# MCG-NJU/LinK

Measured on AMD Instinct MI355X. Metric: voxels/s through one LinK (3x7)^3 block, 100k active voxels C=64, higher is better.
Workload: dtype f32

## Files before the change

link_amd/csrc/dense_common.h:

```cpp
#pragma once
#include <limits.h>

#include "elk_common.h"

namespace link {

typedef int v4i_t __attribute__((ext_vector_type(4)));

#define DC_OOB 0xFFFFFFF0u
#ifndef DC_PROF
#define DC_PROF 0
#endif
#define DC_PROF_PTR(p) do { if (!DC_PROF) (p) = nullptr; } while (0)
#define DC_NOW() (DC_PROF == 2 ? __builtin_amdgcn_s_memrealtime() : __builtin_amdgcn_s_memtime())
#ifndef DC_ST_AUX
#define DC_ST_AUX 16
#endif
__device__ __forceinline__ __amdgpu_buffer_rsrc_t dc_rsrc(const void *base, uint32_t bytes) {
  return __builtin_amdgcn_make_buffer_rsrc(const_cast<void *>(base), 0, bytes, 0x00020000);
}
__device__ __forceinline__ void st16(__amdgpu_buffer_rsrc_t r, uint32_t byte_off, float4 v) {
  const v4i_t x = {__builtin_bit_cast(int, v.x), __builtin_bit_cast(int, v.y), __builtin_bit_cast(int, v.z),
                   __builtin_bit_cast(int, v.w)};
  __builtin_amdgcn_raw_buffer_store_b128(x, r, byte_off, 0, DC_ST_AUX);
}
__device__ __forceinline__ void st16i(__amdgpu_buffer_rsrc_t r, uint32_t byte_off, int4 v) {
  const v4i_t x = {v.x, v.y, v.z, v.w};
  __builtin_amdgcn_raw_buffer_store_b128(x, r, byte_off, 0, 0);
}
__device__ __forceinline__ void st4i(__amdgpu_buffer_rsrc_t r, uint32_t byte_off, int v) {
  __builtin_amdgcn_raw_buffer_store_b32(v, r, byte_off, 0, 0);
}
template <bool COH>
__device__ __forceinline__ void st16i_c(__amdgpu_buffer_rsrc_t r, uint32_t byte_off, int4 v) {
  const v4i_t x = {v.x, v.y, v.z, v.w};
  __builtin_amdgcn_raw_buffer_store_b128(x, r, byte_off, 0, COH ? 16 : 0);
}
template <bool COH>
__device__ __forceinline__ void st4i_c(__amdgpu_buffer_rsrc_t r, uint32_t byte_off, int v) {
  __builtin_amdgcn_raw_buffer_store_b32(v, r, byte_off, 0, COH ? 16 : 0);
}
template <bool COH>
__device__ __forceinline__ int4 ld16i_c(__amdgpu_buffer_rsrc_t r, const int4 *base, uint32_t idx) {
  if constexpr (COH) {
    const v4i_t x = __builtin_amdgcn_raw_buffer_load_b128(r, idx * 16u, 0, 16);
    return make_int4(x.x, x.y, x.z, x.w);
  } else {
    return base[idx];
  }
}
template <bool COH>
__device__ __forceinline__ int ld4i_c(__amdgpu_buffer_rsrc_t r, const uint32_t *base, uint32_t idx) {
  if constexpr (COH) return __builtin_amdgcn_raw_buffer_load_b32(r, idx * 4u, 0, 16);
  else return (int)base[idx];
}

#define DC_STATS_SLOTS 16
__device__ __forceinline__ void dc_index_stats_flush(int32_t *stats, int n_in, int n_first, int mx) {
  __shared__ int s_part[16][3];
#pragma unroll
  for (int o = 32; o > 0; o >>= 1) {
    n_in += __shfl_xor(n_in, o, 64);
    n_first += __shfl_xor(n_first, o, 64);
    mx = max(mx, __shfl_xor(mx, o, 64));
  }
  const int lane = (int)(threadIdx.x & 63), wave = (int)(threadIdx.x >> 6);
  if (lane == 0) { s_part[wave][0] = n_in; s_part[wave][1] = n_first; s_part[wave][2] = mx; }
  __syncthreads();
  if (threadIdx.x == 0) {
    int a = 0, f = 0, m = 0;
    for (int w = 0; w < (int)(blockDim.x >> 6); w++) { a += s_part[w][0]; f += s_part[w][1]; m = max(m, s_part[w][2]); }
    int32_t *slot = stats + (blockIdx.x % DC_STATS_SLOTS) * 16;
    if (a) atomicAdd(&slot[0], a);
    if (f) atomicAdd(&slot[1], f);
    if (m) atomicMax(&slot[2], m);
  }
}

#ifndef DC_THETA_BOUND
#define DC_THETA_BOUND 1
#endif
__device__ __forceinline__ void dc_coord_absmax(const link_dc_grid_t &g, float coord_div, float &ax, float &ay, float &az) {
  float a[3];
#pragma unroll
  for (int k = 0; k < 3; k++) {
    const float lo = (float)g.lo[k] * (float)g.s, hi = ((float)g.lo[k] + (float)g.dim[k]) * (float)g.s;
    a[k] = fmaxf(fabsf(lo), fabsf(hi)) / coord_div;
  }
  ax = a[0]; ay = a[1]; az = a[2];
}
__device__ __forceinline__ bool dc_theta_leaves_fast_range(float ax, float ay, float az, float w0, float w1, float w2, float alpha) {
  const float b = (fabsf(w0) * ax + fabsf(w1) * ay + fabsf(w2) * az) * fabsf(alpha) * 1.01f;
  return !(b < 32768.0f);
}

__device__ __forceinline__ int dc_cell(const link_dc_grid_t &g, int ux, int uy, int uz, int ub) {
  return ((ub * g.pdim[0] + ux + 1) * g.pdim[1] + uy + 1) * g.pdim[2] + uz + 1;
}

#define DC_INL 4
__device__ __forceinline__ uint32_t dc_slot(const link_dc_grid_t &g, int pcell, int rank) {
  return rank < DC_INL ? (uint32_t)pcell * DC_INL + (uint32_t)rank
                       : (uint32_t)g.vp * DC_INL + (uint32_t)pcell * (uint32_t)(g.k - DC_INL) + (uint32_t)(rank - DC_INL);
}

template <bool STATS, bool COH = false>
__device__ __forceinline__ void dc_index_body(const int4 *__restrict__ coords, int64_t n, const link_dc_grid_t &g,
                                              uint32_t *__restrict__ cnt, int4 *__restrict__ slots,
                                              int32_t *__restrict__ vcell, int32_t *__restrict__ hdr, int bid, int nblk,
                                              int nthr, int &st_in, int &st_first, int &st_max) {
  const __amdgpu_buffer_rsrc_t r_slots = dc_rsrc(slots, (uint32_t)((int64_t)g.vp * g.k * 16));
  const __amdgpu_buffer_rsrc_t r_cnt = dc_rsrc(cnt, (uint32_t)(g.vp * 4));
  if (bid == 0 && threadIdx.x == 0) hdr[LINK_HDR_NVALID] = (int32_t)n;
  for (int64_t v = (int64_t)bid * nthr + threadIdx.x; v < n; v += (int64_t)nblk * nthr) {
    const int4 rc = coords[v];
    const unsigned ux = (unsigned)(floordiv(rc.x, g.s) - g.lo[0]), uy = (unsigned)(floordiv(rc.y, g.s) - g.lo[1]);
    const unsigned uz = (unsigned)(floordiv(rc.z, g.s) - g.lo[2]), ub = (unsigned)(rc.w - g.lo[3]);
    const bool inside = ux < (unsigned)g.dim[0] && uy < (unsigned)g.dim[1] && uz < (unsigned)g.dim[2] &&
                        ub < (unsigned)g.dim[3];
    if (!inside) atomicOr(&hdr[LINK_HDR_STATUS_ACC], 1);
    const int pcell = inside ? dc_cell(g, (int)ux, (int)uy, (int)uz, (int)ub) : 0;
    const int rank = __builtin_amdgcn_raw_ptr_buffer_atomic_add_i32(1, r_cnt, pcell ? (uint32_t)pcell * 4u : DC_OOB, 0, 0);
    const bool full = pcell != 0 && rank >= g.k;
    if (full) atomicOr(&hdr[LINK_HDR_STATUS_ACC], 2);
    const bool keep = pcell != 0 && !full;
    st16i_c<COH>(r_slots, keep ? dc_slot(g, pcell, rank) * 16u : DC_OOB, make_int4(rc.x, rc.y, rc.z, (int)v));
    vcell[v] = keep ? pcell : 0;
    if (STATS) { st_in += pcell != 0; st_first += (pcell != 0 && rank == 0); st_max = max(st_max, pcell != 0 ? rank + 1 : 0); }
  }
}

#define DC_SID_INL 8
__device__ __forceinline__ uint32_t dc_sid_off(const link_dc_grid_t &g, int pcell, int rank) {
  const int kk = g.k > DC_SID_INL ? g.k - DC_SID_INL : 0;
  return rank < DC_SID_INL ? (uint32_t)pcell * DC_SID_INL + (uint32_t)rank
                           : (uint32_t)g.vp * DC_SID_INL + (uint32_t)pcell * (uint32_t)kk + (uint32_t)(rank - DC_SID_INL);
}

template <int N>
__device__ __forceinline__ void wait_vmcnt() {
  asm volatile("s_waitcnt vmcnt(%0)" ::"n"(N) : "memory");
}

static inline bool dc_width_ok(int c) { return c == 16 || c == 32 || c == 64 || c == 128; }

}
```

link_amd/csrc/dense_fused_impl.h:

```cpp
#pragma once
#include <type_traits>

#include "dense_gather.h"
#include "dense_io.h"

namespace DC_IO_NS {
using namespace link;

#include "dense_k1_impl.h"

template <int C, int OP, int NB, bool PIPE, bool WB = true>
static int launch_k1p(const link_dc_buffers_t *b, const link_dc_grid_t &g, const link_elk_desc_t &d, int64_t n,
                     bool warm, hipStream_t st) {
  using K = dc_k1_cfg<C, OP>;
  const int64_t vi = (int64_t)g.dim[0] * g.dim[1] * g.dim[2] * g.dim[3];
  int64_t waves = (int64_t)(b->tune.k1_wgs > 0 ? b->tune.k1_wgs : 512) * 4;
  int cpw = (int)((vi + waves - 1) / waves);
  if (cpw < 1) cpw = 1;
  const int64_t wgs = (vi + (int64_t)cpw * K::NW - 1) / ((int64_t)cpw * K::NW);
  int k1_pad = b->tune.k1_lds_pad;
  k1_pad = k1_pad < 0 ? 0 : (k1_pad > 16384 ? 16384 : k1_pad);
  const int lds_k1 = K::LDS_BYTES + k1_pad <= 160 * 1024 ? K::LDS_BYTES + k1_pad : K::LDS_BYTES;
  if (lds_k1 > 64 * 1024)
    (void)hipFuncSetAttribute(reinterpret_cast<const void *>(&k_dc_premix_modsum<C, OP, NB, PIPE, WB>),
                              hipFuncAttributeMaxDynamicSharedMemorySize, lds_k1);
  hipLaunchKernelGGL((k_dc_premix_modsum<C, OP, NB, PIPE, WB>), dim3((unsigned)wgs), dim3(64 * K::NW), lds_k1, st, b->feats,
                     reinterpret_cast<int4 *>(b->slots), b->cnt, b->cell_n, b->w_pre, b->pre_ln_w, b->pre_ln_b,
                     b->w_pos, b->alpha, d.cg, d.coord_div, d.eps, n, g, cpw, warm, b->S, b->fin, b->hdr,
                     reinterpret_cast<unsigned long long *>(b->tune.k1_dbg));
  return check_launch("link_dc_premix_modsum");
}

template <int C, int OP, int NB>
static int launch_k1(const link_dc_buffers_t *b, const link_dc_grid_t &g, const link_elk_desc_t &d, int64_t n,
                     bool warm, bool wb, hipStream_t st) {
  if constexpr (C == 64 && NB == 2 && OP != LINK_OP_COSX) {
    if (!wb) return launch_k1p<C, OP, NB, false, false>(b, g, d, n, warm, st);
  }
  return launch_k1p<C, OP, NB, false>(b, g, d, n, warm, st);
}

template <int C, int OP>
static int dispatch_k1_nb(const link_dc_buffers_t *b, const link_dc_grid_t &g, const link_elk_desc_t &d, int64_t n,
                          bool warm, bool wb, hipStream_t st) {
  constexpr int T = C / 16;
  int nb = (d.cg % 16 == 0) ? d.cg / 16 : T;
  if (nb > T) nb = T;
  if (nb == T) return launch_k1<C, OP, T>(b, g, d, n, warm, wb, st);
  if (T >= 2 && nb == T / 2) return launch_k1<C, OP, (T >= 2 ? T / 2 : 1)>(b, g, d, n, warm, wb, st);
  if (T >= 4 && nb == T / 4) return launch_k1<C, OP, (T >= 4 ? T / 4 : 1)>(b, g, d, n, warm, wb, st);
  return launch_k1<C, OP, T>(b, g, d, n, warm, wb, st);
}

template <int C>
static int dispatch_k1_op(const link_dc_buffers_t *b, const link_dc_grid_t &g, const link_elk_desc_t &d, int64_t n,
                          bool warm, bool wb, hipStream_t st) {
  switch (d.op) {
    case LINK_OP_COS: return dispatch_k1_nb<C, LINK_OP_COS>(b, g, d, n, warm, wb, st);
    case LINK_OP_SIN: return dispatch_k1_nb<C, LINK_OP_SIN>(b, g, d, n, warm, wb, st);
    default: return dispatch_k1_nb<C, LINK_OP_COSX>(b, g, d, n, warm, wb, st);
  }
}

#include "dense_fused_mm_impl.h"

template <int LPR, int OP, bool PAIR, bool DIV>
__global__ void __launch_bounds__(256) k_dc_demod(const float *__restrict__ A_, const float *__restrict__ fin,
                                                  const int4 *__restrict__ coords, const int32_t *__restrict__ vcell,
                                                  const float *__restrict__ w_pos, const float *__restrict__ alpha,
                                                  const float *__restrict__ ln_w, const float *__restrict__ ln_b, int c,
                                                  int cg, float coord_div, float eps, int64_t n, int64_t a_rows,
                                                  void *__restrict__ out) {
  constexpr int P = (OP == LINK_OP_COSX) ? 3 : 2;
  constexpr int G = 64 / LPR;
  const int lane = threadIdx.x & 63;
  const int li = lane & (LPR - 1);
  const int ch0 = 4 * li;
  const bool hi = PAIR && (li >= LPR / 2);
  const int ra = P * c * 4;
  const __amdgpu_buffer_rsrc_t r_A = dc_rsrc(A_, (uint32_t)(a_rows * ra));
  const __amdgpu_buffer_rsrc_t r_fin = dc_rsrc(fin, (uint32_t)(n * c * 4));
  const __amdgpu_buffer_rsrc_t r_out = dc_rsrc(out, (uint32_t)(n * c * IO_BYTES));
  float w0[4], w1[4], w2[4], al[4], gw[4], gb[4];
#pragma unroll
  for (int e = 0; e < 4; e++) {
    const int ch = ch0 + e, tc = ch % cg;
    w0[e] = w_pos[3 * tc + 0]; w1[e] = w_pos[3 * tc + 1]; w2[e] = w_pos[3 * tc + 2];
    al[e] = alpha ? alpha[tc] : 1.0f;
    gw[e] = ln_w[ch]; gb[e] = ln_b[ch];
  }
  const float inv_c = 1.0f / (float)c;
  const int64_t npair = (n + 1) >> 1;
  const int64_t ngroups = (int64_t)gridDim.x * 4 * G;
  int64_t p = ((int64_t)blockIdx.x * 4 + (threadIdx.x >> 6)) * G + lane / LPR;
  if (p >= npair) return;
  auto ld_meta = [&](int64_t pp, int4 &ca, int4 &cb, int &va, int &vb) {
    const int64_t q = pp < npair ? pp : npair - 1;
    const int64_t ia = 2 * q, ib = (2 * q + 1 < n) ? 2 * q + 1 : 2 * q;
    ca = coords[ia]; cb = coords[ib];
    va = vcell[ia]; vb = vcell[ib];
  };
  auto ld_rows = [&](int va, int vb, v4i_t (&ra_)[P], v4i_t (&rb_)[P]) {
#pragma unroll
    for (int pp = 0; pp < P; pp++) {
      ra_[pp] = __builtin_amdgcn_raw_buffer_load_b128(r_A, (uint32_t)va * (uint32_t)ra + (uint32_t)((pp * c + ch0) * 4), 0, 0);
      rb_[pp] = __builtin_amdgcn_raw_buffer_load_b128(r_A, (uint32_t)vb * (uint32_t)ra + (uint32_t)((pp * c + ch0) * 4), 0, 0);
    }
  };
  int4 c0a, c0b, c1a, c1b;
  int v0a, v0b, v1a, v1b;
  v4i_t a0[P], b0[P];
  ld_meta(p, c0a, c0b, v0a, v0b);
  ld_rows(v0a, v0b, a0, b0);
  ld_meta(p + ngroups, c1a, c1b, v1a, v1b);
  for (; p < npair; p += ngroups) {
    v4i_t a1[P], b1[P];
    ld_rows(v1a, v1b, a1, b1);
    int4 c2a, c2b;
    int v2a, v2b;
    ld_meta(p + 2 * ngroups, c2a, c2b, v2a, v2b);
    const bool hasB = 2 * p + 1 < n;
    v4i_t fx = {0, 0, 0, 0}, fy = {0, 0, 0, 0};
    if (OP == LINK_OP_COSX) {
      fx = __builtin_amdgcn_raw_buffer_load_b128(r_fin, (uint32_t)(2 * p) * (uint32_t)(c * 4) + (uint32_t)(ch0 * 4), 0, 0);
      fy = __builtin_amdgcn_raw_buffer_load_b128(r_fin, hasB ? (uint32_t)(2 * p + 1) * (uint32_t)(c * 4) + (uint32_t)(ch0 * 4) : DC_OOB, 0, 0);
    }
    float nvA[4], nvB[4], sA = 0.f, sB = 0.f;
    float thA[4], thB[4];
    bool big = false;
    {
      const bool swapped = PAIR && hi && hasB;
      float xa = (float)(swapped ? c0b.x : c0a.x), ya = (float)(swapped ? c0b.y : c0a.y), za = (float)(swapped ? c0b.z : c0a.z);
      float xb = (float)c0b.x, yb = (float)c0b.y, zb = (float)c0b.z;
      if (DIV) { xa = xa / coord_div; ya = ya / coord_div; za = za / coord_div; xb = xb / coord_div; yb = yb / coord_div; zb = zb / coord_div; }
#pragma unroll
      for (int e = 0; e < 4; e++) {
        thA[e] = theta_of(xa, ya, za, w0[e], w1[e], w2[e], al[e]);
        thB[e] = PAIR ? thA[e] : theta_of(xb, yb, zb, w0[e], w1[e], w2[e], al[e]);
        big |= !(fabsf(thA[e]) < 32768.0f) || !(fabsf(thB[e]) < 32768.0f);
      }
    }
    float snA[4], csA[4], snB[4], csB[4];
    if (__builtin_expect(__any(big), 0)) {
#pragma unroll
      for (int e = 0; e < 4; e++) {
        sincos_nocall(thA[e], snA[e], csA[e]);
        if (PAIR) { snB[e] = snA[e]; csB[e] = csA[e]; } else sincos_nocall(thB[e], snB[e], csB[e]);
      }
    } else {
#pragma unroll
      for (int e = 0; e < 4; e++) {
        sincos_small(thA[e], snA[e], csA[e]);
        if (PAIR) { snB[e] = snA[e]; csB[e] = csA[e]; } else sincos_small(thB[e], snB[e], csB[e]);
      }
    }
    if (PAIR) {
      const bool swapped = hi && hasB;
#pragma unroll
      for (int e = 0; e < 4; e++) {
        const float sn = snA[e], cs = csA[e];
        const float so = partner<LPR>(sn), co = partner<LPR>(cs);
        snA[e] = swapped ? so : sn; csA[e] = swapped ? co : cs;
        snB[e] = hi ? sn : so;      csB[e] = hi ? cs : co;
      }
    }
#pragma unroll
    for (int e = 0; e < 4; e++) {
      const float A0 = __int_as_float(a0[0][e]), A1 = __int_as_float(a0[1][e]);
      const float B0 = __int_as_float(b0[0][e]), B1 = __int_as_float(b0[1][e]);
      if (OP == LINK_OP_SIN) {
        nvA[e] = __fsub_rn(__fmul_rn(A0, csA[e]), __fmul_rn(A1, snA[e]));
        nvB[e] = __fsub_rn(__fmul_rn(B0, csB[e]), __fmul_rn(B1, snB[e]));
      } else {
        nvA[e] = __fadd_rn(__fmul_rn(A0, csA[e]), __fmul_rn(A1, snA[e]));
        nvB[e] = __fadd_rn(__fmul_rn(B0, csB[e]), __fmul_rn(B1, snB[e]));
      }
      if (OP == LINK_OP_COSX) {
        nvA[e] = __fadd_rn(nvA[e], __fsub_rn(__int_as_float(a0[P - 1][e]), link_mul_rn(__int_as_float(fx[e]), thA[e])));
        nvB[e] = __fadd_rn(nvB[e], __fsub_rn(__int_as_float(b0[P - 1][e]), link_mul_rn(__int_as_float(fy[e]), thB[e])));
      }
      sA += nvA[e]; sB += nvB[e];
    }
    sA = grp_sum<LPR>(sA);
    sB = grp_sum<LPR>(sB);
    const float meanA = sA * inv_c, meanB = sB * inv_c;
    float qA = 0.f, qB = 0.f;
#pragma unroll
    for (int e = 0; e < 4; e++) {
// ... 780 lines not shown
```

link_amd/csrc/dense_k1_impl.h:

```cpp
#pragma once

#ifndef DC_K1_LCAP
#define DC_K1_LCAP 352
#endif
#ifndef DC_K1_NW
#define DC_K1_NW 4
#endif
#ifndef DC_K1_ABL
#define DC_K1_ABL 0
#endif
#ifndef DC_K1_SPLIT
#define DC_K1_SPLIT 1
#endif
#ifndef DC_K2_ABL
#define DC_K2_ABL 0
#endif
#ifndef DC_K2_SECOND_ROUND
#define DC_K2_SECOND_ROUND 1
#endif
#ifndef DC_K2_PIPE_READS
#define DC_K2_PIPE_READS 0
#endif
#ifndef DC_K1_MFMA32
#define DC_K1_MFMA32 1
#endif
#ifndef DC_K1_SUMB
#define DC_K1_SUMB 8
#endif
#ifndef DC_K1_SWAP_SUMS
#define DC_K1_SWAP_SUMS 1
#endif
#ifndef DC_K1_LATE_PUBLISH
#define DC_K1_LATE_PUBLISH 0
#endif
__device__ __forceinline__ float dc_k1_sum_groups(float v) {
#if DC_K1_SWAP_SUMS
  float a = v, b = v;
  asm volatile("s_nop 1\n\tv_permlane32_swap_b32 %0, %1" : "+v"(a), "+v"(b));
  a += b;
  b = a;
  asm volatile("s_nop 1\n\tv_permlane16_swap_b32 %0, %1" : "+v"(a), "+v"(b));
  return a + b;
#else
  v += __shfl_xor(v, 16, 64);
  v += __shfl_xor(v, 32, 64);
  return v;
#endif
}

template <int C, int OP>
struct dc_k1_cfg {
  static constexpr int T = C / 16;
  static constexpr int P = op_parts<OP>::value;
  static constexpr int LDW = C + 4;
  static constexpr int RB = P * C * 4;
  static constexpr int XROW = RB + 16;
  static constexpr int RGL = P * C / 4;
  static constexpr int RGS = RGL <= 8 ? 8 : (RGL <= 16 ? 16 : (RGL <= 32 ? 32 : 64));
  static constexpr int RG = 64 / RGS;
  static constexpr int LCAP = DC_K1_LCAP;
  static constexpr int LDH = 2 * C + 8;
  static constexpr int WIMG_BYTES = DC_K1_SPLIT ? C * LDH * 2 : C * LDW * 4;
  static constexpr int W_BYTES = WIMG_BYTES + (2 * C + 4 * C) * 4;
  static constexpr int LIST_OFF = 0;
  static constexpr int SCELL_OFF = LCAP * 16;
  static constexpr int X_OFF = SCELL_OFF + LCAP * 4;
  static constexpr int WAVE_BYTES = X_OFF + 16 * XROW;
  static constexpr int NW = DC_K1_NW;
  static constexpr int LDS_BYTES = W_BYTES + NW * WAVE_BYTES;
};


#ifndef DC_K1_WAVES
#define DC_K1_WAVES 2
#endif
__device__ __forceinline__ int dc_k1_cell_of(const link_dc_grid_t &g, int chunk, int nrem, int lane) {
  const int q = chunk + (lane < nrem ? lane : 0);
  const int Dx = g.dim[0], Dy = g.dim[1], Dz = g.dim[2];
  const int z = q % Dz;
  int t = q / Dz;
  const int y = t % Dy;
  t /= Dy;
  return dc_cell(g, t % Dx, y, z, t / Dx);
}

template <bool COH = false>
__device__ __forceinline__ void dc_k1_prefetch(int &pc_f, int &nv_f, int4 &rf0, int4 &rf1, int4 &rf2, int4 &rf3,
                                               const link_dc_grid_t &g, const int4 *__restrict__ slots,
                                               const uint32_t *__restrict__ csrc, int c_begin, int c_end, int lane) {
  pc_f = 0; nv_f = 0;
  rf0 = make_int4(0, 0, 0, 0); rf1 = rf0; rf2 = rf0; rf3 = rf0;
  if (c_begin < c_end) {
    pc_f = dc_k1_cell_of(g, c_begin, (c_end - c_begin < 64) ? c_end - c_begin : 64, lane);
    const __amdgpu_buffer_rsrc_t r_slots = dc_rsrc(slots, (uint32_t)((int64_t)g.vp * g.k * 16));
    const __amdgpu_buffer_rsrc_t r_c = dc_rsrc(csrc, (uint32_t)(g.vp * 4));
    rf0 = ld16i_c<COH>(r_slots, slots, (uint32_t)pc_f * DC_INL + 0); rf1 = ld16i_c<COH>(r_slots, slots, (uint32_t)pc_f * DC_INL + 1);
    rf2 = ld16i_c<COH>(r_slots, slots, (uint32_t)pc_f * DC_INL + 2); rf3 = ld16i_c<COH>(r_slots, slots, (uint32_t)pc_f * DC_INL + 3);
    nv_f = ld4i_c<COH>(r_c, csrc, (uint32_t)pc_f);
  }
}

template <int C, int OP>
__device__ __forceinline__ void dc_k1_stage(char *smem_raw, const float *__restrict__ w_pre, const float *__restrict__ ln_w,
                                            const float *__restrict__ ln_b, const float *__restrict__ w_pos,
                                            const float *__restrict__ alpha, int cg, float coord_div, const link_dc_grid_t &g,
                                            int tid, bool &w_big, bool &th_big) {
  using K = dc_k1_cfg<C, OP>;
  constexpr int LDW = K::LDW;
  float *w_lds = reinterpret_cast<float *>(smem_raw);
  float *ln_lds = reinterpret_cast<float *>(smem_raw + K::WIMG_BYTES);
  float *pw_lds = ln_lds + 2 * C;
  (void)w_lds;
  {
    constexpr int NF4 = C * C / 4;
    constexpr int NT = 64 * K::NW;
    constexpr int NV = (NF4 + NT - 1) / NT;
    float4 wv[NV];
#pragma unroll
    for (int i = 0; i < NV; i++) {
      const int e = (i * NT + tid) * 4;
      wv[i] = *reinterpret_cast<const float4 *>(&w_pre[(NF4 % NT == 0 || e < C * C) ? e : 0]);
    }
#pragma unroll
    for (int i = 0; i < NV; i++) {
      int e = (i * NT + tid) * 4;
      if (NF4 % NT != 0 && e >= C * C) e = 0;
      const int r = e / C, col = e - r * C;
      const float4 wq = (NF4 % NT == 0 || (i * NT + tid) * 4 < C * C) ? wv[i] : *reinterpret_cast<const float4 *>(&w_pre[0]);
      if constexpr (DC_K1_SPLIT) {
        uint2 hi, lo;
        dc_split4(wq, hi, lo);
        unsigned short *wh = reinterpret_cast<unsigned short *>(smem_raw);
        *reinterpret_cast<uint2 *>(&wh[r * K::LDH + col]) = hi;
        *reinterpret_cast<uint2 *>(&wh[r * K::LDH + C + col]) = lo;
        w_big |= !(fmaxf(fmaxf(fabsf(wq.x), fabsf(wq.y)), fmaxf(fabsf(wq.z), fabsf(wq.w))) < 32768.0f);
      } else {
        *reinterpret_cast<float4 *>(&w_lds[r * LDW + col]) = wq;
      }
    }
    if (tid < C) ln_lds[tid] = ln_w[tid];
    else if (tid < 2 * C) ln_lds[tid] = ln_b[tid - C];
    if (tid < C) {
      const int tc = tid % cg;
      const float q0 = w_pos[3 * tc + 0], q1 = w_pos[3 * tc + 1], q2 = w_pos[3 * tc + 2], qa = alpha ? alpha[tc] : 1.0f;
      pw_lds[tid] = q0; pw_lds[C + tid] = q1; pw_lds[2 * C + tid] = q2;
      pw_lds[3 * C + tid] = qa;
      if (DC_THETA_BOUND) {
        float ax, ay, az;
        dc_coord_absmax(g, coord_div, ax, ay, az);
        th_big = dc_theta_leaves_fast_range(ax, ay, az, q0, q1, q2, qa);
      }
    }
  }
}

template <int C, int OP, int NB, bool PIPE, bool COH = false, bool WB = true>
__device__ __forceinline__ void dc_k1_range(char *smem_raw, const void *__restrict__ feats, int4 *__restrict__ slots,
                                            uint32_t *__restrict__ cnt, int32_t *__restrict__ cell_n,
                                            const float *__restrict__ w_pre, float coord_div, float eps, int64_t n,
                                            const link_dc_grid_t &g, bool warm, float *__restrict__ S_, float *__restrict__ fin,
                                            unsigned long long *__restrict__ dbg, int c_begin,
                                            int c_end, const int pc_f, const int nv_f, const int4 rf0, const int4 rf1, const int4 rf2,
                                            const int4 rf3, bool w_big, bool th_slow, int wid,
                                            unsigned long long tq0, unsigned long long tq1) {
  using K = dc_k1_cfg<C, OP>;
  constexpr int T = K::T, P = K::P, LDW = K::LDW;
  unsigned long long tq_cell = 0, tq_fill = 0, tq_body = 0, tq_sum = 0;
  int tq_tiles = 0;
  float *w_lds = reinterpret_cast<float *>(smem_raw);
  float *ln_lds = reinterpret_cast<float *>(smem_raw + K::WIMG_BYTES);
  float *pw_lds = ln_lds + 2 * C;
  const int tid = threadIdx.x, lane = tid & 63, wave = __builtin_amdgcn_readfirstlane(tid >> 6);
  const int li = lane & 15, gq = lane >> 4;
  char *wbase = smem_raw + K::W_BYTES + wave * K::WAVE_BYTES;
  int4 *list = reinterpret_cast<int4 *>(wbase + K::LIST_OFF);
  int *scell = reinterpret_cast<int *>(wbase + K::SCELL_OFF);
  char *xbuf = wbase + K::X_OFF;
  const uint32_t *__restrict__ csrc = warm ? reinterpret_cast<const uint32_t *>(cell_n) : cnt;
  const __amdgpu_buffer_rsrc_t r_S = dc_rsrc(S_, (uint32_t)((g.vp + 1) * K::RB));
  const __amdgpu_buffer_rsrc_t r_fin = dc_rsrc(fin, (uint32_t)(n * C * 4));
  const __amdgpu_buffer_rsrc_t r_slots = dc_rsrc(slots, (uint32_t)((int64_t)g.vp * g.k * 16));
  const __amdgpu_buffer_rsrc_t r_n = dc_rsrc(cell_n, (uint32_t)(g.vp * 4));
  const __amdgpu_buffer_rsrc_t r_cnt = dc_rsrc(cnt, (uint32_t)(g.vp * 4));
  const int rl = lane;
  const bool ract = rl < K::RGL;

  for (int chunk = c_begin; chunk < c_end;) {
    const int nrem = (c_end - chunk < 64) ? c_end - chunk : 64;
    unsigned long long tqa = dbg ? DC_NOW() : 0;
    int pc, nv;
    int4 r0, r1, r2, r3;
    if (chunk == c_begin) {
      pc = pc_f; nv = nv_f; r0 = rf0; r1 = rf1; r2 = rf2; r3 = rf3;
    } else {
      pc = dc_k1_cell_of(g, chunk, nrem, lane);
      r0 = ld16i_c<COH>(r_slots, slots, (uint32_t)pc * DC_INL + 0); r1 = ld16i_c<COH>(r_slots, slots, (uint32_t)pc * DC_INL + 1);
      r2 = ld16i_c<COH>(r_slots, slots, (uint32_t)pc * DC_INL + 2); r3 = ld16i_c<COH>(r_slots, slots, (uint32_t)pc * DC_INL + 3);
      nv = ld4i_c<COH>(warm ? r_n : r_cnt, csrc, (uint32_t)pc);
    }
    constexpr int LCAPX = K::LCAP;
    nv = nv < g.k ? nv : g.k;
    nv = nv < LCAPX ? nv : LCAPX;
    if (lane >= nrem) nv = 0;
    int incl = nv;
    incl += __builtin_amdgcn_update_dpp(0, incl, 0x111, 0xF, 0xF, true);
    incl += __builtin_amdgcn_update_dpp(0, incl, 0x112, 0xF, 0xF, true);
    incl += __builtin_amdgcn_update_dpp(0, incl, 0x114, 0xF, 0xF, true);
    incl += __builtin_amdgcn_update_dpp(0, incl, 0x118, 0xF, 0xF, true);
    {
      const int t0 = __builtin_amdgcn_readlane(incl, 15), t1 = __builtin_amdgcn_readlane(incl, 31), t2 = __builtin_amdgcn_readlane(incl, 47);
      incl += gq == 0 ? 0 : (gq == 1 ? t0 : (gq == 2 ? t0 + t1 : t0 + t1 + t2));
    }
    const unsigned long long fit = __ballot(lane < nrem && incl <= LCAPX);
    const int nfit = __builtin_amdgcn_readfirstlane(__popcll(fit));
    const int Ttot = __builtin_amdgcn_readlane(incl, nfit - 1);
    int4 rs[4] = {r0, r1, r2, r3};
    if (lane < nfit) {
      const int excl = incl - nv;
      int k0 = nv > 0 ? r0.w * 4 + 0 : INT_MAX, k1 = nv > 1 ? r1.w * 4 + 1 : INT_MAX;
      int k2 = nv > 2 ? r2.w * 4 + 2 : INT_MAX, k3 = nv > 3 ? r3.w * 4 + 3 : INT_MAX;
      int a, bb;
      a = min(k0, k1); bb = max(k0, k1); k0 = a; k1 = bb;
      a = min(k2, k3); bb = max(k2, k3); k2 = a; k3 = bb;
      a = min(k0, k2); bb = max(k0, k2); k0 = a; k2 = bb;
      a = min(k1, k3); bb = max(k1, k3); k1 = a; k3 = bb;
      a = min(k1, k2); bb = max(k1, k2); k1 = a; k2 = bb;
      const int ks[4] = {k0, k1, k2, k3};
#pragma unroll
      for (int j = 0; j < 4; j++) {
        const int s = ks[j] & 3;
        int4 r;
        r.x = s == 0 ? r0.x : (s == 1 ? r1.x : (s == 2 ? r2.x : r3.x));
        r.y = s == 0 ? r0.y : (s == 1 ? r1.y : (s == 2 ? r2.y : r3.y));
        r.z = s == 0 ? r0.z : (s == 1 ? r1.z : (s == 2 ? r2.z : r3.z));
        r.w = ks[j] >> 2;
        if (j < nv) { list[excl + j] = r; scell[excl + j] = pc; }
        rs[j] = r;
      }
      for (int k = DC_INL; k < nv; k++) {
        const int4 r = ld16i_c<COH>(r_slots, slots, dc_slot(g, pc, k));
        scell[excl + k] = pc;
        int pos = k;
        while (pos > 0 && list[excl + pos - 1].w > r.w) {
          list[excl + pos] = list[excl + pos - 1];
          pos--;
        }
        list[excl + pos] = r;
      }
      if constexpr (WB) {
        if (nv > DC_INL && !warm)
          for (int k = 0; k < nv; k++) st16i_c<COH>(r_slots, dc_slot(g, pc, k) * 16u, list[excl + k]);
      }
    }
    auto publish = [&]() {
      if constexpr (WB) {
#pragma unroll
        for (int j = 0; j < 4; j++)
          st16i_c<COH>(r_slots, (lane < nfit && j < nv && nv <= DC_INL && !warm) ? ((uint32_t)pc * DC_INL + j) * 16u : DC_OOB, rs[j]);
      }
      const uint32_t coff = (lane < nfit && !warm) ? (uint32_t)pc * 4u : DC_OOB;
      st4i_c<COH>(r_n, coff, nv);
      st4i(r_cnt, coff, 0);
    };
    auto publish_empty = [&]() {
      for (unsigned long long em = __ballot(lane < nfit && nv == 0); em; em &= em - 1) {
        const int pcj = __builtin_amdgcn_readlane(pc, __builtin_ctzll(em));
        st16(r_S, ract ? (uint32_t)pcj * (uint32_t)K::RB + (uint32_t)rl * 16u : DC_OOB, make_float4(0.f, 0.f, 0.f, 0.f));
      }
    };
    if constexpr (!DC_K1_LATE_PUBLISH) { publish(); publish_empty(); }
    __builtin_amdgcn_wave_barrier();
    asm volatile("s_waitcnt lgkmcnt(0)" ::: "memory");
    if (dbg) { const unsigned long long tqb = DC_NOW(); tq_cell += tqb - tqa; tqa = tqb; }
    const int ntile = (Ttot + 15) >> 4;
    const int nloop = ntile;
    float4 acc = make_float4(0.f, 0.f, 0.f, 0.f);
    auto ld_rows = [&](int tile_idx, int4 &rr, float4 (&ff)[T]) {
      int sl = 16 * tile_idx + li;
      sl = sl < Ttot ? sl : Ttot - 1;
      rr = list[sl];
#pragma unroll
      for (int tt = 0; tt < T; tt++)
        ff[tt] = io_ld4(feats, (int64_t)((DC_K1_ABL & 8) ? li : rr.w) * C + 16 * tt + 4 * gq);
    };
    auto mfma_tile = [&](const float4 (&ff)[T], floatx4 (&cc)[T]) {
      if (DC_K1_ABL & 1) {
#pragma unroll
        for (int tp = 0; tp < T; tp++) cc[tp] = (floatx4){ff[tp].x, ff[tp].y, ff[tp].z, ff[tp].w};
        return;
      }
#pragma unroll
      for (int tp = 0; tp < T; tp++) cc[tp] = (floatx4){0.f, 0.f, 0.f, 0.f};
      if constexpr (DC_K1_SPLIT) {
        uint2 bh[T], bl[T];
        float mx = 0.f;
#pragma unroll
        for (int tt = 0; tt < T; tt++) {
          dc_split4(ff[tt], bh[tt], bl[tt]);
          mx = fmaxf(mx, fmaxf(fmaxf(fabsf(ff[tt].x), fabsf(ff[tt].y)), fmaxf(fabsf(ff[tt].z), fabsf(ff[tt].w))));
        }
        if (__builtin_expect(!(w_big || __any(!(mx < 32768.0f))), 1)) {
          const unsigned short *wh = reinterpret_cast<const unsigned short *>(smem_raw);
          if constexpr (DC_K1_MFMA32 && T % 2 == 0) {
#pragma unroll
            for (int tt = 0; tt < T; tt += 2) {
              uint2 ah[2][T], al[2][T];
#pragma unroll
              for (int h = 0; h < 2; h++)
#pragma unroll
                for (int tp = 0; tp < T; tp++) {
                  ah[h][tp] = *reinterpret_cast<const uint2 *>(&wh[(16 * tp + li) * K::LDH + 16 * (tt + h) + 4 * gq]);
                  al[h][tp] = *reinterpret_cast<const uint2 *>(&wh[(16 * tp + li) * K::LDH + C + 16 * (tt + h) + 4 * gq]);
                }
#pragma unroll
              for (int tp = 0; tp < T; tp++) cc[tp] = dc_mfma_f16x2(al[0][tp], al[1][tp], bh[tt], bh[tt + 1], cc[tp]);
              if constexpr (IO != 1) {
#pragma unroll
                for (int tp = 0; tp < T; tp++) cc[tp] = dc_mfma_f16x2(ah[0][tp], ah[1][tp], bl[tt], bl[tt + 1], cc[tp]);
              }
#pragma unroll
              for (int tp = 0; tp < T; tp++) cc[tp] = dc_mfma_f16x2(ah[0][tp], ah[1][tp], bh[tt], bh[tt + 1], cc[tp]);
            }
            return;
          }
#pragma unroll
          for (int tt = 0; tt < T; tt++) {
            uint2 ah[T], al[T];
#pragma unroll
            for (int tp = 0; tp < T; tp++) {
              ah[tp] = *reinterpret_cast<const uint2 *>(&wh[(16 * tp + li) * K::LDH + 16 * tt + 4 * gq]);
              al[tp] = *reinterpret_cast<const uint2 *>(&wh[(16 * tp + li) * K::LDH + C + 16 * tt + 4 * gq]);
            }
#pragma unroll
            for (int tp = 0; tp < T; tp++) cc[tp] = dc_mfma_f16(al[tp], bh[tt], cc[tp]);
            if constexpr (IO != 1) {
#pragma unroll
              for (int tp = 0; tp < T; tp++) cc[tp] = dc_mfma_f16(ah[tp], bl[tt], cc[tp]);
            }
#pragma unroll
            for (int tp = 0; tp < T; tp++) cc[tp] = dc_mfma_f16(ah[tp], bh[tt], cc[tp]);
          }
          return;
        }
      }
#pragma unroll
      for (int tt = 0; tt < T; tt++) {
        float4 a[T];
#pragma unroll
        for (int tp = 0; tp < T; tp++) {
          if constexpr (DC_K1_SPLIT) a[tp] = *reinterpret_cast<const float4 *>(&w_pre[(16 * tp + li) * C + 16 * tt + 4 * gq]);
          else a[tp] = *reinterpret_cast<const float4 *>(&w_lds[(16 * tp + li) * LDW + 16 * tt + 4 * gq]);
        }
#pragma unroll
        for (int tp = 0; tp < T; tp++) cc[tp] = __builtin_amdgcn_mfma_f32_16x16x4f32(a[tp].x, ff[tt].x, cc[tp], 0, 0, 0);
#pragma unroll
        for (int tp = 0; tp < T; tp++) cc[tp] = __builtin_amdgcn_mfma_f32_16x16x4f32(a[tp].y, ff[tt].y, cc[tp], 0, 0, 0);
#pragma unroll
        for (int tp = 0; tp < T; tp++) cc[tp] = __builtin_amdgcn_mfma_f32_16x16x4f32(a[tp].z, ff[tt].z, cc[tp], 0, 0, 0);
#pragma unroll
        for (int tp = 0; tp < T; tp++) cc[tp] = __builtin_amdgcn_mfma_f32_16x16x4f32(a[tp].w, ff[tt].w, cc[tp], 0, 0, 0);
      }
    };
    int4 recA = make_int4(0, 0, 0, 0), recB = recA, recC = recA;
    float4 fA[T], fB[T];
    floatx4 acA[T], acB[T];
    if (ntile > 0) {
      ld_rows(0, recA, PIPE ? fB : fA);
      ld_rows(ntile > 1 ? 1 : 0, recB, PIPE ? fA : fB);
      if constexpr (DC_K1_LATE_PUBLISH) publish();
      mfma_tile(PIPE ? fB : fA, acA);
    } else {
      if constexpr (DC_K1_LATE_PUBLISH) publish();
    }
    if constexpr (DC_K1_LATE_PUBLISH) publish_empty();
    if (dbg) { const unsigned long long tqb = DC_NOW(); tq_fill += tqb - tqa; tqa = tqb; }
    auto step = [&](auto phase_tag, int t, const int4 &rec, const int4 &recn, int4 &rec2, const float4 (&fn)[T], float4 (&f2)[T],
                    const floatx4 (&ac)[T], floatx4 (&acn)[T]) {
      constexpr int PHASE = decltype(phase_tag)::value;
      if (PHASE != 2 && ntile > 0) {
        const int slot = 16 * t + li;
        float x = (float)rec.x, y = (float)rec.y, z = (float)rec.z;
        if (coord_div != 1.0f) { x = x / coord_div; y = y / coord_div; z = z / coord_div; }
        float th[NB][4];
        bool big = false;
#pragma unroll
        for (int tb = 0; tb < NB; tb++) {
          const float4 q0 = *reinterpret_cast<const float4 *>(&pw_lds[16 * tb + 4 * gq]);
          const float4 q1 = *reinterpret_cast<const float4 *>(&pw_lds[C + 16 * tb + 4 * gq]);
          const float4 q2 = *reinterpret_cast<const float4 *>(&pw_lds[2 * C + 16 * tb + 4 * gq]);
          const float4 qa = *reinterpret_cast<const float4 *>(&pw_lds[3 * C + 16 * tb + 4 * gq]);
          th[tb][0] = theta_of(x, y, z, q0.x, q1.x, q2.x, qa.x); th[tb][1] = theta_of(x, y, z, q0.y, q1.y, q2.y, qa.y);
          th[tb][2] = theta_of(x, y, z, q0.z, q1.z, q2.z, qa.z); th[tb][3] = theta_of(x, y, z, q0.w, q1.w, q2.w, qa.w);
          if (!DC_THETA_BOUND) {
#pragma unroll
            for (int r = 0; r < 4; r++) big |= !(fabsf(th[tb][r]) < 32768.0f);
          }
        }
        const bool slow = DC_THETA_BOUND ? th_slow : __any(big);
        const bool more = PIPE && t + 1 < ntile;
        (void)recn;
        auto body = [&](auto more_tag, auto slow_tag) {
          constexpr bool MORE = decltype(more_tag)::value, SLOW = decltype(slow_tag)::value;
          if constexpr (MORE) mfma_tile(fn, acn);
          if constexpr (MORE) ld_rows(t + 2 < ntile ? t + 2 : t + 1, rec2, f2);
          float sn[NB][4], cs[NB][4];
#pragma unroll
          for (int tb = 0; tb < NB; tb++)
#pragma unroll
            for (int r = 0; r < 4; r++) {
              if (DC_K1_ABL & 2) { sn[tb][r] = th[tb][r]; cs[tb][r] = 1.0f - th[tb][r]; }
              else if constexpr (SLOW) sincos_nocall(th[tb][r], sn[tb][r], cs[tb][r]);
              else sincos_small(th[tb][r], sn[tb][r], cs[tb][r]);
            }
          float s = 0.f;
#pragma unroll
          for (int tp = 0; tp < T; tp++) s += (ac[tp][0] + ac[tp][1]) + (ac[tp][2] + ac[tp][3]);
          s = dc_k1_sum_groups(s);
          const float mean = s * (1.0f / C);
          float qq = 0.f;
#pragma unroll
          for (int tp = 0; tp < T; tp++)
#pragma unroll
            for (int r = 0; r < 4; r++) {
              const float d = ac[tp][r] - mean;
              qq += d * d;
            }
          qq = dc_k1_sum_groups(qq);
          const float rstd = 1.0f / sqrtf(qq * (1.0f / C) + eps);
#pragma unroll
          for (int tp = 0; tp < T; tp++) {
            const float4 lw = *reinterpret_cast<const float4 *>(&ln_lds[16 * tp + 4 * gq]);
            const float4 lb = *reinterpret_cast<const float4 *>(&ln_lds[C + 16 * tp + 4 * gq]);
            const float fv[4] = {(ac[tp][0] - mean) * rstd * lw.x + lb.x, (ac[tp][1] - mean) * rstd * lw.y + lb.y,
                                 (ac[tp][2] - mean) * rstd * lw.z + lb.z, (ac[tp][3] - mean) * rstd * lw.w + lb.w};
            if (OP == LINK_OP_COSX)
              st16(r_fin, slot < Ttot ? (uint32_t)rec.w * (uint32_t)(C * 4) + (uint32_t)((16 * tp + 4 * gq) * 4) : DC_OOB,
                   make_float4(fv[0], fv[1], fv[2], fv[3]));
            const int tb = tp % NB;
            float p0[4], p1[4], p2[4];
#pragma unroll
            for (int r = 0; r < 4; r++) {
              if (OP == LINK_OP_SIN) { p0[r] = fv[r] * sn[tb][r]; p1[r] = fv[r] * cs[tb][r]; }
              else { p0[r] = fv[r] * cs[tb][r]; p1[r] = fv[r] * sn[tb][r]; }
              p2[r] = fv[r] * th[tb][r];
            }
            char *xr = xbuf + li * K::XROW + (16 * tp + 4 * gq) * 4;
            *reinterpret_cast<float4 *>(xr) = make_float4(p0[0], p0[1], p0[2], p0[3]);
            *reinterpret_cast<float4 *>(xr + C * 4) = make_float4(p1[0], p1[1], p1[2], p1[3]);
            if (P == 3) *reinterpret_cast<float4 *>(xr + 2 * C * 4) = make_float4(p2[0], p2[1], p2[2], p2[3]);
          }
          if constexpr (MORE && !SLOW) {
#pragma unroll
            for (int i = 0; i < T * T * 4; i++) {
              __builtin_amdgcn_sched_group_barrier(0x008, 1, 0);
              __builtin_amdgcn_sched_group_barrier(0x002, 6, 0);
            }
          }
        };
        if (__builtin_expect(slow, 0)) {
          if (more) {
            mfma_tile(fn, acn);
            ld_rows(t + 2 < ntile ? t + 2 : t + 1, rec2, f2);
          }
          body(std::false_type{}, std::true_type{});
        } else {
          if (more) body(std::true_type{}, std::false_type{}); else body(std::false_type{}, std::false_type{});
        }
        __builtin_amdgcn_wave_barrier();
        asm volatile("s_waitcnt lgkmcnt(0)" ::: "memory");
      }
      if (PHASE != 2 && dbg) { const unsigned long long tqb = DC_NOW(); tq_body += tqb - tqa; tqa = tqb; tq_tiles++; }
      if (PHASE == 1 || (DC_K1_ABL & 4)) return;
      {
        const int slot = 16 * t + li;
        const int myc = slot < Ttot ? scell[slot] : -1;
        const int nxc = slot + 1 < Ttot ? scell[slot + 1] : -2;
        const unsigned closes = (unsigned)__ballot(gq == 0 && slot < Ttot && myc != nxc);
        const char *xrow = xbuf + (ract ? rl : 0) * 16;
#pragma unroll
        for (int h = 0; h < 16; h += DC_K1_SUMB) {
          float4 v[DC_K1_SUMB];
#pragma unroll
          for (int k = 0; k < DC_K1_SUMB; k++) v[k] = *reinterpret_cast<const float4 *>(xrow + (h + k) * K::XROW);
#pragma unroll
          for (int k = 0; k < DC_K1_SUMB; k++) {
            if (16 * t + h + k < Ttot) {
              acc.x += v[k].x; acc.y += v[k].y; acc.z += v[k].z; acc.w += v[k].w;
              if ((closes >> (h + k)) & 1u) {
                const int pcs = __builtin_amdgcn_readlane(myc, h + k);
                st16(r_S, ract ? (uint32_t)pcs * (uint32_t)K::RB + (uint32_t)rl * 16u : DC_OOB, acc);
                acc = make_float4(0.f, 0.f, 0.f, 0.f);
              }
            }
          }
        }
      }
      __builtin_amdgcn_wave_barrier();
      if (dbg) { const unsigned long long tqb = DC_NOW(); tq_sum += tqb - tqa; tqa = tqb; }
    };
    if constexpr (PIPE) {
      for (int t = 0; t < nloop; t += 2) {
        step(std::integral_constant<int, 0>{}, t, recA, recB, recC, fA, fB, acA, acB);
        recA = recB; recB = recC;
        if (t + 1 < nloop) {
          step(std::integral_constant<int, 0>{}, t + 1, recA, recB, recC, fB, fA, acB, acA);
          recA = recB; recB = recC;
        }
      }
    } else {
      using body_only = std::integral_constant<int, 1>;
      using sums_only = std::integral_constant<int, 2>;
      for (int t = 0; t < nloop; t += 2) {
        if (t > 0) {
          if (t + 1 < ntile) ld_rows(t + 1, recB, fB);
          mfma_tile(fA, acA);
        }
        if (t > 0) step(sums_only{}, t - 1, recB, recB, recC, fB, fB, acA, acB);
        step(body_only{}, t, recA, recB, recC, fB, fB, acA, acB);
        if (t + 1 < nloop) {
          if (t + 2 < ntile) ld_rows(t + 2, recA, fA);
          mfma_tile(fB, acA);
          step(sums_only{}, t, recA, recA, recC, fA, fA, acA, acB);
          step(body_only{}, t + 1, recB, recA, recC, fA, fA, acA, acB);
        }
      }
      if (nloop > 0) step(sums_only{}, nloop - 1, recA, recA, recC, fA, fA, acA, acB);
    }
    chunk += nfit;
  }
  if (dbg && lane == 0) {
    unsigned long long *d = dbg + (size_t)wid * 8;
    const unsigned long long te = DC_NOW();
    d[0] = tq1 - tq0; d[1] = tq_cell; d[2] = tq_fill; d[3] = tq_body; d[4] = tq_sum; d[5] = te - tq0; d[6] = tq_tiles; d[7] = tq0;
  }
}

template <int C, int OP, int NB, bool PIPE, bool WB = true>
__global__ void __launch_bounds__(64 * DC_K1_NW, PIPE ? 2 : DC_K1_WAVES) k_dc_premix_modsum(
    const void *__restrict__ feats, int4 *__restrict__ slots, uint32_t *__restrict__ cnt,
    int32_t *__restrict__ cell_n, const float *__restrict__ w_pre, const float *__restrict__ ln_w,
    const float *__restrict__ ln_b, const float *__restrict__ w_pos, const float *__restrict__ alpha, int cg,
    float coord_div, float eps, int64_t n, link_dc_grid_t g, int cpw, bool warm, float *__restrict__ S_,
    float *__restrict__ fin, int32_t *__restrict__ hdr, unsigned long long *__restrict__ dbg) {
  using K = dc_k1_cfg<C, OP>;
  DC_PROF_PTR(dbg);
  unsigned long long tq0 = dbg ? DC_NOW() : 0, tq1 = 0;
  extern __shared__ __attribute__((aligned(16))) char smem_raw[];
  const int tid = threadIdx.x, lane = tid & 63, wave = __builtin_amdgcn_readfirstlane(tid >> 6);
  const int Vi = g.dim[0] * g.dim[1] * g.dim[2] * g.dim[3];
  const int wid = blockIdx.x * K::NW + wave;
  const int c_begin = wid * cpw;
  const int c_end = (c_begin + cpw < Vi) ? c_begin + cpw : Vi;
  int pc_f, nv_f;
  int4 rf0, rf1, rf2, rf3;
  dc_k1_prefetch<false>(pc_f, nv_f, rf0, rf1, rf2, rf3, g, slots, warm ? reinterpret_cast<const uint32_t *>(cell_n) : cnt, c_begin, c_end, lane);
  bool w_big = false;
  bool th_big = false;
  dc_k1_stage<C, OP>(smem_raw, w_pre, ln_w, ln_b, w_pos, alpha, cg, coord_div, g, tid, w_big, th_big);
  if (blockIdx.x == 0 && tid == 0 && !warm) {
    hdr[LINK_HDR_STATUS] = hdr[LINK_HDR_STATUS_ACC];
    hdr[LINK_HDR_STATUS_ACC] = 0;
  }
  w_big = DC_K1_SPLIT ? (__syncthreads_or(w_big) != 0 || (LINK_COSX_EXACT && OP == LINK_OP_COSX)) : (__syncthreads(), false);
  const bool th_slow = DC_THETA_BOUND ? __syncthreads_or(th_big) != 0 : false;
  if (dbg) tq1 = DC_NOW();
  if (c_begin >= c_end) return;
  dc_k1_range<C, OP, NB, PIPE, false, WB>(smem_raw, feats, slots, cnt, cell_n, w_pre, coord_div, eps, n, g, warm, S_, fin, dbg, c_begin,
                                       c_end, pc_f, nv_f, rf0, rf1, rf2, rf3, w_big, th_slow, wid, tq0, tq1);
}
```

Before: 3.319 billion.

## Restructure per-cell row summation into lane-sliced running accumulation with ballot-driven stores

Replaces the grouped row-sum reduction of the modulated sums with a scheme where each lane owns a fixed byte slice of the row and keeps a running accumulator across slots. It stores that slice to the cell's S row whenever a ballot shows the cell closes. The old path stays reachable through a new RS template flag selected by a tuning bit. The change also prefetches the LayerNorm weight and bias before the reductions, adds an asm barrier to keep the summation order fixed, and makes the tail row loads unconditional by clamping the tile index. The aim is to cut cross-lane reduction and LDS traffic in the sum phase, at the cost of more registers and serial per-row adds.

```diff
diff --git a/link_amd/csrc/dense_common.h b/link_amd/csrc/dense_common.h
--- a/link_amd/csrc/dense_common.h
+++ b/link_amd/csrc/dense_common.h
@@ -23,6 +23,19 @@
   const v4i_t x = {__builtin_bit_cast(int, v.x), __builtin_bit_cast(int, v.y), __builtin_bit_cast(int, v.z),
                    __builtin_bit_cast(int, v.w)};
   __builtin_amdgcn_raw_buffer_store_b128(x, r, byte_off, 0, DC_ST_AUX);
+}
+typedef int dc_v2i_t __attribute__((ext_vector_type(2)));
+__device__ __forceinline__ void st16(__amdgpu_buffer_rsrc_t r, uint32_t byte_off, uint32_t row_off, float4 v) {
+  const v4i_t x = {__builtin_bit_cast(int, v.x), __builtin_bit_cast(int, v.y), __builtin_bit_cast(int, v.z),
+                   __builtin_bit_cast(int, v.w)};
+  __builtin_amdgcn_raw_buffer_store_b128(x, r, byte_off, row_off, DC_ST_AUX);
+}
+__device__ __forceinline__ void st8(__amdgpu_buffer_rsrc_t r, uint32_t byte_off, uint32_t row_off, float2 v) {
+  const dc_v2i_t x = {__builtin_bit_cast(int, v.x), __builtin_bit_cast(int, v.y)};
+  __builtin_amdgcn_raw_buffer_store_b64(x, r, byte_off, row_off, DC_ST_AUX);
+}
+__device__ __forceinline__ void st4f(__amdgpu_buffer_rsrc_t r, uint32_t byte_off, uint32_t row_off, float v) {
+  __builtin_amdgcn_raw_buffer_store_b32(__builtin_bit_cast(int, v), r, byte_off, row_off, DC_ST_AUX);
 }
 __device__ __forceinline__ void st16i(__amdgpu_buffer_rsrc_t r, uint32_t byte_off, int4 v) {
   const v4i_t x = {v.x, v.y, v.z, v.w};
diff --git a/link_amd/csrc/dense_fused_impl.h b/link_amd/csrc/dense_fused_impl.h
--- a/link_amd/csrc/dense_fused_impl.h
+++ b/link_amd/csrc/dense_fused_impl.h
@@ -9,7 +9,7 @@
 
 #include "dense_k1_impl.h"
 
-template <int C, int OP, int NB, bool PIPE, bool WB = true>
+template <int C, int OP, int NB, bool PIPE, bool WB = true, bool RS = false>
 static int launch_k1p(const link_dc_buffers_t *b, const link_dc_grid_t &g, const link_elk_desc_t &d, int64_t n,
                      bool warm, hipStream_t st) {
   using K = dc_k1_cfg<C, OP>;
@@ -22,9 +22,9 @@
   k1_pad = k1_pad < 0 ? 0 : (k1_pad > 16384 ? 16384 : k1_pad);
   const int lds_k1 = K::LDS_BYTES + k1_pad <= 160 * 1024 ? K::LDS_BYTES + k1_pad : K::LDS_BYTES;
   if (lds_k1 > 64 * 1024)
-    (void)hipFuncSetAttribute(reinterpret_cast<const void *>(&k_dc_premix_modsum<C, OP, NB, PIPE, WB>),
+    (void)hipFuncSetAttribute(reinterpret_cast<const void *>(&k_dc_premix_modsum<C, OP, NB, PIPE, WB, RS>),
                               hipFuncAttributeMaxDynamicSharedMemorySize, lds_k1);
-  hipLaunchKernelGGL((k_dc_premix_modsum<C, OP, NB, PIPE, WB>), dim3((unsigned)wgs), dim3(64 * K::NW), lds_k1, st, b->feats,
+  hipLaunchKernelGGL((k_dc_premix_modsum<C, OP, NB, PIPE, WB, RS>), dim3((unsigned)wgs), dim3(64 * K::NW), lds_k1, st, b->feats,
                      reinterpret_cast<int4 *>(b->slots), b->cnt, b->cell_n, b->w_pre, b->pre_ln_w, b->pre_ln_b,
                      b->w_pos, b->alpha, d.cg, d.coord_div, d.eps, n, g, cpw, warm, b->S, b->fin, b->hdr,
                      reinterpret_cast<unsigned long long *>(b->tune.k1_dbg));
@@ -34,6 +34,9 @@
 template <int C, int OP, int NB>
 static int launch_k1(const link_dc_buffers_t *b, const link_dc_grid_t &g, const link_elk_desc_t &d, int64_t n,
                      bool warm, bool wb, hipStream_t st) {
+  if constexpr (C == 64 || (C == 32 && OP == LINK_OP_COS)) {
+    if (b->tune.k1_form & 32) return launch_k1p<C, OP, NB, false, true, true>(b, g, d, n, warm, st);
+  }
   if constexpr (C == 64 && NB == 2 && OP != LINK_OP_COSX) {
     if (!wb) return launch_k1p<C, OP, NB, false, false>(b, g, d, n, warm, st);
   }
diff --git a/link_amd/csrc/dense_k1_impl.h b/link_amd/csrc/dense_k1_impl.h
--- a/link_amd/csrc/dense_k1_impl.h
+++ b/link_amd/csrc/dense_k1_impl.h
@@ -56,8 +56,8 @@
   static constexpr int RB = P * C * 4;
   static constexpr int XROW = RB + 16;
   static constexpr int RGL = P * C / 4;
-  static constexpr int RGS = RGL <= 8 ? 8 : (RGL <= 16 ? 16 : (RGL <= 32 ? 32 : 64));
-  static constexpr int RG = 64 / RGS;
+  static constexpr int PB = (P == 2 && C >= 32) ? RB / 64 : 16;
+  static constexpr int NPL = RB / PB;
   static constexpr int LCAP = DC_K1_LCAP;
   static constexpr int LDH = 2 * C + 8;
   static constexpr int WIMG_BYTES = DC_K1_SPLIT ? C * LDH * 2 : C * LDW * 4;
@@ -154,7 +154,7 @@
   }
 }
 
-template <int C, int OP, int NB, bool PIPE, bool COH = false, bool WB = true>
+template <int C, int OP, int NB, bool PIPE, bool COH = false, bool WB = true, bool RS = false>
 __device__ __forceinline__ void dc_k1_range(char *smem_raw, const void *__restrict__ feats, int4 *__restrict__ slots,
                                             uint32_t *__restrict__ cnt, int32_t *__restrict__ cell_n,
                                             const float *__restrict__ w_pre, float coord_div, float eps, int64_t n,
@@ -184,6 +184,19 @@
   const __amdgpu_buffer_rsrc_t r_cnt = dc_rsrc(cnt, (uint32_t)(g.vp * 4));
   const int rl = lane;
   const bool ract = rl < K::RGL;
+  constexpr int PB = K::PB, NA = PB / 4;
+  const bool pact = lane < K::NPL;
+  const uint32_t pvo = pact ? (uint32_t)lane * (uint32_t)PB : DC_OOB;
+  auto ld_piece = [](const char *p, float (&o)[NA]) {
+    if constexpr (NA == 4) { const float4 q = *reinterpret_cast<const float4 *>(p); o[0] = q.x; o[1] = q.y; o[2] = q.z; o[3] = q.w; }
+    else if constexpr (NA == 2) { const float2 q = *reinterpret_cast<const float2 *>(p); o[0] = q.x; o[1] = q.y; }
+    else o[0] = *reinterpret_cast<const float *>(p);
+  };
+  auto st_piece = [&](uint32_t row_off, const float (&a)[NA]) {
+    if constexpr (NA == 4) st16(r_S, pvo, row_off, make_float4(a[0], a[1], a[2], a[3]));
+    else if constexpr (NA == 2) st8(r_S, pvo, row_off, make_float2(a[0], a[1]));
+    else st4f(r_S, pvo, row_off, a[0]);
+  };
 
   for (int chunk = c_begin; chunk < c_end;) {
     const int nrem = (c_end - chunk < 64) ? c_end - chunk : 64;
@@ -275,6 +288,9 @@
     const int ntile = (Ttot + 15) >> 4;
     const int nloop = ntile;
     float4 acc = make_float4(0.f, 0.f, 0.f, 0.f);
+    float accp[NA];
+#pragma unroll
+    for (int e = 0; e < NA; e++) accp[e] = 0.f;
     auto ld_rows = [&](int tile_idx, int4 &rr, float4 (&ff)[T]) {
       int sl = 16 * tile_idx + li;
       sl = sl < Ttot ? sl : Ttot - 1;
@@ -412,9 +428,21 @@
               else if constexpr (SLOW) sincos_nocall(th[tb][r], sn[tb][r], cs[tb][r]);
               else sincos_small(th[tb][r], sn[tb][r], cs[tb][r]);
             }
+          constexpr int TH = T >= 4 ? T / 2 : T;
+          float4 lw[T], lb[T];
+#pragma unroll
+          for (int tp = 0; tp < TH; tp++) {
+            lw[tp] = *reinterpret_cast<const float4 *>(&ln_lds[16 * tp + 4 * gq]);
+            lb[tp] = *reinterpret_cast<const float4 *>(&ln_lds[C + 16 * tp + 4 * gq]);
+          }
           float s = 0.f;
 #pragma unroll
-          for (int tp = 0; tp < T; tp++) s += (ac[tp][0] + ac[tp][1]) + (ac[tp][2] + ac[tp][3]);
+          for (int tp = 0; tp < T; tp++) {
+            float u = ac[tp][0] + ac[tp][1];
+            const float w = ac[tp][2] + ac[tp][3];
+            asm("" : "+v"(u));
+            s += u + w;
+          }
           s = dc_k1_sum_groups(s);
           const float mean = s * (1.0f / C);
           float qq = 0.f;
@@ -428,11 +456,14 @@
           qq = dc_k1_sum_groups(qq);
           const float rstd = 1.0f / sqrtf(qq * (1.0f / C) + eps);
 #pragma unroll
+          for (int tp = TH; tp < T; tp++) {
+            lw[tp] = *reinterpret_cast<const float4 *>(&ln_lds[16 * tp + 4 * gq]);
+            lb[tp] = *reinterpret_cast<const float4 *>(&ln_lds[C + 16 * tp + 4 * gq]);
+          }
+#pragma unroll
           for (int tp = 0; tp < T; tp++) {
-            const float4 lw = *reinterpret_cast<const float4 *>(&ln_lds[16 * tp + 4 * gq]);
-            const float4 lb = *reinterpret_cast<const float4 *>(&ln_lds[C + 16 * tp + 4 * gq]);
-            const float fv[4] = {(ac[tp][0] - mean) * rstd * lw.x + lb.x, (ac[tp][1] - mean) * rstd * lw.y + lb.y,
-                                 (ac[tp][2] - mean) * rstd * lw.z + lb.z, (ac[tp][3] - mean) * rstd * lw.w + lb.w};
+            const float fv[4] = {(ac[tp][0] - mean) * rstd * lw[tp].x + lb[tp].x, (ac[tp][1] - mean) * rstd * lw[tp].y + lb[tp].y,
+                                 (ac[tp][2] - mean) * rstd * lw[tp].z + lb[tp].z, (ac[tp][3] - mean) * rstd * lw[tp].w + lb[tp].w};
             if (OP == LINK_OP_COSX)
               st16(r_fin, slot < Ttot ? (uint32_t)rec.w * (uint32_t)(C * 4) + (uint32_t)((16 * tp + 4 * gq) * 4) : DC_OOB,
                    make_float4(fv[0], fv[1], fv[2], fv[3]));
@@ -471,7 +502,7 @@
       }
       if (PHASE != 2 && dbg) { const unsigned long long tqb = DC_NOW(); tq_body += tqb - tqa; tqa = tqb; tq_tiles++; }
       if (PHASE == 1 || (DC_K1_ABL & 4)) return;
-      {
+      if constexpr (RS || K::PB == 16) {
         const int slot = 16 * t + li;
         const int myc = slot < Ttot ? scell[slot] : -1;
         const int nxc = slot + 1 < Ttot ? scell[slot + 1] : -2;
@@ -494,6 +525,36 @@
             }
           }
         }
+      } else {
+        const int slot = 16 * t + li;
+        const int c0 = scell[slot], c1 = scell[slot + 1];
+        const int myc = slot < Ttot ? c0 : -1;
+        const int nxc = slot + 1 < Ttot ? c1 : -2;
+        const unsigned closes = (unsigned)__ballot(gq == 0 && slot < Ttot && myc != nxc);
+        const uint32_t crow = (uint32_t)myc * (uint32_t)K::RB;
+        const char *xrow = xbuf + (pact ? lane : 0) * PB;
+        auto rows = [&](auto full_tag) {
+          constexpr bool FULL = decltype(full_tag)::value;
+#pragma unroll
+          for (int h = 0; h < 16; h += DC_K1_SUMB) {
+            float v[DC_K1_SUMB][NA];
+#pragma unroll
+            for (int k = 0; k < DC_K1_SUMB; k++) ld_piece(xrow + (h + k) * K::XROW, v[k]);
+#pragma unroll
+            for (int k = 0; k < DC_K1_SUMB; k++) {
+              if (FULL || 16 * t + h + k < Ttot) {
+#pragma unroll
+                for (int e = 0; e < NA; e++) accp[e] += v[k][e];
+                if ((closes >> (h + k)) & 1u) {
+                  st_piece((uint32_t)__builtin_amdgcn_readlane((int)crow, h + k), accp);
+#pragma unroll
+                  for (int e = 0; e < NA; e++) accp[e] = 0.f;
+                }
+              }
+            }
+          }
+        };
+        if (16 * t + 16 <= Ttot) rows(std::true_type{}); else rows(std::false_type{});
       }
       __builtin_amdgcn_wave_barrier();
       if (dbg) { const unsigned long long tqb = DC_NOW(); tq_sum += tqb - tqa; tqa = tqb; }
@@ -512,13 +573,13 @@
       using sums_only = std::integral_constant<int, 2>;
       for (int t = 0; t < nloop; t += 2) {
         if (t > 0) {
-          if (t + 1 < ntile) ld_rows(t + 1, recB, fB);
+          ld_rows(t + 1 < ntile ? t + 1 : ntile - 1, recB, fB);
           mfma_tile(fA, acA);
         }
         if (t > 0) step(sums_only{}, t - 1, recB, recB, recC, fB, fB, acA, acB);
         step(body_only{}, t, recA, recB, recC, fB, fB, acA, acB);
         if (t + 1 < nloop) {
-          if (t + 2 < ntile) ld_rows(t + 2, recA, fA);
+          ld_rows(t + 2 < ntile ? t + 2 : ntile - 1, recA, fA);
           mfma_tile(fB, acA);
           step(sums_only{}, t, recA, recA, recC, fA, fA, acA, acB);
           step(body_only{}, t + 1, recB, recA, recC, fA, fA, acA, acB);
@@ -535,7 +596,7 @@
   }
 }
 
-template <int C, int OP, int NB, bool PIPE, bool WB = true>
+template <int C, int OP, int NB, bool PIPE, bool WB = true, bool RS = false>
 __global__ void __launch_bounds__(64 * DC_K1_NW, PIPE ? 2 : DC_K1_WAVES) k_dc_premix_modsum(
     const void *__restrict__ feats, int4 *__restrict__ slots, uint32_t *__restrict__ cnt,
     int32_t *__restrict__ cell_n, const float *__restrict__ w_pre, const float *__restrict__ ln_w,
@@ -565,6 +626,6 @@
   const bool th_slow = DC_THETA_BOUND ? __syncthreads_or(th_big) != 0 : false;
   if (dbg) tq1 = DC_NOW();
   if (c_begin >= c_end) return;
-  dc_k1_range<C, OP, NB, PIPE, false, WB>(smem_raw, feats, slots, cnt, cell_n, w_pre, coord_div, eps, n, g, warm, S_, fin, dbg, c_begin,
+  dc_k1_range<C, OP, NB, PIPE, false, WB, RS>(smem_raw, feats, slots, cnt, cell_n, w_pre, coord_div, eps, n, g, warm, S_, fin, dbg, c_begin,
                                        c_end, pc_f, nv_f, rf0, rf1, rf2, rf3, w_big, th_slow, wid, tq0, tq1);
 }
```

After: 3.394 billion, median of 6. About the same (+2.3%).
